# omuses/hqp

Hardware: AMD Instinct MI355X
Metric: KKT factor+solve/sec (fp64) (higher is better)
Workload: dtype f64; 1 GPU; C4 = BASELINE configs[3], the metric's 10^6-variable DOCP: multistage LQ optimal control QP, K=200 stages, nx=5000 states, nu=50 controls -> n=1015000 me=1005000 m=20000, dense fx/fu handed over as blocks, x_0 fixed, box bounds on u; plugin LQDOCP (STAGED engine), one system per GPU; stages=200, nx=5000, nu=50, n=1015000, me=1005000, m=20000, plugin=LQDOCP, kkt_dim_full=2040000

## Files before the change

### hqp_amd/_lib.py

```python
from __future__ import annotations

import ctypes as C
import os

import numpy as np

_HERE = os.path.dirname(os.path.abspath(__file__))
LIB_PATH = os.environ.get("HQPKKT_LIB") or os.path.join(_HERE, "libhqpkkt.so")

OK, E_SIZES, E_MEM, E_SING, E_FORMAT, E_NULL, E_RANGE, E_INTERN, E_DEVICE = 0, 1, 3, 4, 6, 8, 10, 17, 100
MODE_FULL, MODE_REDUCED, MODE_STAGED = 0, 1, 2
LOC_HOST, LOC_DEVICE = 0, 1
DYN_DENSE, DYN_SPARSE, DYN_PROFILE = 0, 1, 3
HESS_CSR, HESS_DENSE = 0, 1
HQPKKT_HESS_UPDATE_RANK = 4
HQPKKT_BFGS_REPORT = 8
HQPKKT_EIG_MAX_STEPS = 128
HQPKKT_EIG_REPORT = 10
HQPKKT_EIG_END_REL = 2.0 ** -40

SYMBOLS = [
    "hqpkkt_default_opts", "hqpkkt_create", "hqpkkt_destroy", "hqpkkt_analyze",
    "hqpkkt_set_values", "hqpkkt_factor", "hqpkkt_step", "hqpkkt_residual", "hqpkkt_solve",
    "hqpkkt_get_sbw", "hqpkkt_get_perm", "hqpkkt_set_tol", "hqpkkt_set_eps",
# ... 4 lines not shown
    "hqpkkt_set_stages", "hqpkkt_debug_stage_ranks", "hqpkkt_debug_stage_block", "hqpkkt_debug_dgemm", "hqpkkt_debug_dgemm2", "hqpkkt_debug_dgemm_full", "hqpkkt_debug_sk_table", "hqpkkt_debug_gemm_form",
    "hqpkkt_analyze_staged", "hqpkkt_set_values_staged", "hqpkkt_set_shard_stream",
    "hqpkkt_values_staging", "hqpkkt_detect_stages", "hqpkkt_stage_staging", "hqpkkt_set_stage_block",
    "hqpkkt_debug_factor_block", "hqpkkt_debug_solve_top_stamps", "hqpkkt_set_dynamics_form", "hqpkkt_set_dense_columns",
    "hqpkkt_debug_sk_profile", "hqpkkt_debug_gemv_profile",
    "hqpkkt_set_packed_panels", "hqpkkt_debug_dgemm_packed", "hqpkkt_debug_gemv_packed", "hqpkkt_debug_carried_packed",
    "hqpkkt_set_dense_rows", "hqpkkt_debug_dgemm_ctrl_rows", "hqpkkt_debug_sk_ctrl_rows",
    "hqpkkt_set_hessian_form", "hqpkkt_set_stage_hessian", "hqpkkt_debug_stage_hessian", "hqpkkt_debug_hess_symv",
    "hqpkkt_set_packed_hessians", "hqpkkt_debug_hess_symv_timed",
    "hqpkkt_update_stage_hessians", "hqpkkt_hessian_product",
    "hqpkkt_bfgs_update_stage_hessians", "hqpkkt_bfgs_report",
    "hqpkkt_hessian_row_stats", "hqpkkt_restart_stage_hessians", "hqpkkt_gerschgorin_stage_hessians",
    "hqpkkt_eigen_control_stage_hessians", "hqpkkt_eigen_report",
    "hqpkkt_debug_gemm_schedule",
    "hqpkkt_debug_gemv_dense", "hqpkkt_debug_symv", "hqpkkt_debug_symv_batch", "hqpkkt_debug_symv_map",
    "hqpkkt_debug_rows_gemv",
]
RCCL_LIB_PATH = os.path.join(_HERE, "libhqpkkt_rccl.so")
RCCL_SYMBOLS = ["hqpkkt_rccl_unique_id", "hqpkkt_rccl_create", "hqpkkt_rccl_create_from_env",
                "hqpkkt_rccl_comm_info", "hqpkkt_rccl_exchange", "hqpkkt_rccl_destroy", "hqpkkt_rccl_origin"]

XCHG_ALLGATHER, XCHG_ALLREDUCE_SUM, XCHG_BCAST_BASE = 0, 1, 16
EXCHANGE_FN = C.CFUNCTYPE(C.c_int, C.c_void_p, C.c_int, C.c_void_p, C.c_longlong, C.c_int)


class Opts(C.Structure):
    _fields_ = [("mode", C.c_int), ("device", C.c_int), ("loc", C.c_int), ("tol", C.c_double),
                ("eps", C.c_double), ("pivot_eps", C.c_double), ("leaf_size", C.c_int),
                ("max_pivots", C.c_int), ("zd_policy", C.c_int), ("slack_policy", C.c_int),
                ("no_small_fronts", C.c_int), ("upd_pingpong_mb", C.c_int), ("amalgamation", C.c_int),
                ("ordering", C.c_int)]
# ... 169 lines not shown
    L.hqpkkt_debug_stage_block.argtypes = [vp, C.c_int, vp, C.c_longlong, C.POINTER(C.c_longlong)]
    L.hqpkkt_debug_dgemm2.argtypes = [C.c_int] * 8 + [C.POINTER(C.c_double)] * 2 + [C.POINTER(C.c_longlong)]
    L.hqpkkt_debug_dgemm_full.argtypes = [C.c_int, C.POINTER(DgemmCase)]
    L.hqpkkt_debug_sk_table.argtypes = [C.c_longlong, C.c_int, C.c_int, C.c_int, C.POINTER(C.c_int), C.c_longlong, C.POINTER(C.c_longlong),
                                        C.POINTER(C.c_int), C.POINTER(C.c_int)]
    L.hqpkkt_debug_dgemm_ctrl_rows.argtypes = [C.c_int, C.POINTER(CtrlRowsCase)]
    L.hqpkkt_debug_sk_ctrl_rows.argtypes = [C.c_int] * 5 + [C.POINTER(C.c_int), C.c_longlong, C.POINTER(C.c_int), C.POINTER(C.c_longlong)]
    L.hqpkkt_debug_sk_profile.argtypes = [C.POINTER(C.c_int), C.c_longlong, C.c_int, C.POINTER(C.c_int), C.c_longlong, C.POINTER(C.c_longlong)]
    L.hqpkkt_debug_gemv_profile.argtypes = [C.c_int] * 4 + [vp, C.c_longlong, C.c_longlong, vp, vp, vp, C.c_double, vp]
    L.hqpkkt_debug_dgemm_packed.argtypes = [C.c_int, C.POINTER(DgemmCase), vp, C.c_longlong, vp]
    L.hqpkkt_debug_gemv_packed.argtypes = [C.c_int] * 4 + [vp, C.c_longlong, vp, vp, vp, vp, C.c_double, vp]
    L.hqpkkt_debug_carried_packed.argtypes = [C.c_int] * 4 + [vp, C.c_longlong, C.c_longlong, vp, C.c_longlong, vp, vp, vp] + [C.c_longlong] * 4
    L.hqpkkt_debug_gemm_form.argtypes = [C.c_int] * 7 + [C.c_longlong] * 3 + [C.c_int, C.POINTER(C.c_longlong)] + [C.POINTER(C.c_int)] * 3
    L.hqpkkt_debug_gemm_schedule.argtypes = [C.POINTER(GemmCaps), C.POINTER(GemmLaunch), C.POINTER(GemmLaunch), C.POINTER(GemmScheduleOut),
                                             C.POINTER(C.c_int), C.c_longlong, C.POINTER(C.c_int), C.c_longlong]
    L.hqpkkt_debug_gemv_dense.argtypes = [C.c_int, C.c_int, C.POINTER(GemvCase)]
    L.hqpkkt_debug_rows_gemv.argtypes = [C.c_int, C.c_int, C.POINTER(RowsCase)]
    L.hqpkkt_debug_symv.argtypes = [C.c_int, C.POINTER(GemvCase)]
    L.hqpkkt_debug_symv_batch.argtypes = [C.c_int, C.c_int, C.POINTER(GemvCase), vp, C.c_longlong, vp, C.c_longlong, C.c_int, C.c_int]
    L.hqpkkt_debug_symv_map.restype = C.c_longlong
    L.hqpkkt_debug_symv_map.argtypes = [C.c_int, C.POINTER(C.c_int), C.c_longlong]
    L.hqpkkt_debug_solve_top_stamps.argtypes = [vp, vp, C.c_int]
    L.hqpkkt_debug_factor_block.argtypes = [C.c_int, C.c_int, vp, C.c_double, C.c_double, C.c_int, C.c_int] + [vp] * 7
    _lib = L
    return L


_rccl = None


# ... 18 lines not shown
```

### hqp_amd/csrc/gemm_form.hpp

```cpp
#pragma once
#include <algorithm>

namespace stg {

static const int GEMM_BK = 16;

static inline long long gemm_tiles(int M, int N, int b, int lower) {
  const long long tm = (M + b - 1) / b, tn = (N + b - 1) / b;
  return lower ? tn * (tn + 1) / 2 + (tm > tn ? (tm - tn) * tn : 0) : tm * tn;
}
static inline long long gemm_slabs(int K) { return (K + GEMM_BK - 1) / GEMM_BK; }

static inline bool gemm_big_tiles(int M, int N, int lower, int K = 0) {
  const long long t = gemm_tiles(M, N, 128, lower);
  return t >= 384 || (!lower && t >= 160 && t <= 256 && K >= 256 * GEMM_BK);
}

static inline bool gemm_use_split_tiles(long long tiles, long long nslab, int grid) {
  if (grid <= 0 || nslab < 32) return false;
  return !(tiles % grid == 0 || tiles >= 16LL * grid);
}
static inline bool gemm_use_split(int M, int N, int K, int lower, int grid) {
  if ((long long)M * N < 256LL * 256) return false;
  const long long tiles = gemm_tiles(M, N, 128, lower);
  if (!gemm_use_split_tiles(tiles, gemm_slabs(K), grid)) return false;
  return tiles > grid * 5 / 8;
// ... 66 lines not shown
```

### hqp_amd/csrc/staged_gemm.hip.h

```cpp
#pragma once
#include <hip/hip_runtime.h>

#include <algorithm>
#include <vector>

#include "gemm_schedule.hpp"

namespace stg {

using kktdev::double4_t;
using kktdev::mfma_f64;

typedef double double2_t __attribute__((ext_vector_type(2)));

struct StripTab {
  int nranks;
  int cut[17];
  int ld[17];
  long long off[17];
};
struct RectTab {
  int nranks;
  int cut[17];
  struct Block {
// ... 52 lines not shown

__device__ __forceinline__ int xcd_swizzle(int bid, int nwg) {
  const int q = nwg >> 3, r = nwg & 7, x = bid & 7;
  return x * q + (x < r ? x : r) + (bid >> 3);
}

template <int BM, int BN, int WGM = 2, int WGN = 2>
struct GemmTile {
  static constexpr int BK = GEMM_BK;
  static constexpr int NW = WGM * WGN, NT = 64 * NW;
  static constexpr int LDA = BM + 16, LDB = BN + 16;
  static constexpr int WM = BM / WGM, WN = BN / WGN, TM = WM / 16, TN = WN / 16;
  static constexpr int LA = BK * BM / 2 / 256, LB = BK * BN / 2 / 256;
  static constexpr int RA = 256 / (BM / 2), RB = 256 / (BN / 2);

  static __device__ __forceinline__ void tile_of(const GemmArgs &g, int t, int &tm, int &tn) {
    if (g.tile_map && BM == 128) {
      const int e = g.tile_map[t];
      tm = e >> 16, tn = e & 0xffff;
    } else if (g.lower) {
      const int tcols = (g.N + BN - 1) / BN, tri = tcols * (tcols + 1) / 2;
      if (t < tri) {
        tm = (int)((sqrtf(8.0f * (float)t + 1.0f) - 1.0f) * 0.5f);
        while ((tm + 1) * (tm + 2) / 2 <= t) tm++;
        while (tm * (tm + 1) / 2 > t) tm--;
        tn = t - tm * (tm + 1) / 2;
      } else {
        tm = tcols + (t - tri) / tcols;
        tn = (t - tri) % tcols;
      }
// ... 106 lines not shown
      }
    }
  }

  static __device__ __forceinline__ void glds16(const double *src, double *lds_row) {
    __builtin_amdgcn_global_load_lds((const __attribute__((address_space(1))) void *)src,
                                     (__attribute__((address_space(3))) void *)lds_row, 16, 0, 0);
  }
  struct Rows {
    int K, k0, k1;
    long long ld, o2, ld2;
  };
  static __device__ __forceinline__ const double *row_of(const Rows &r, const double *p, const double *zr, int k) {
    return k < r.K ? p + (long long)k * r.ld : (k >= r.k0 && k < r.k1) ? p + (r.o2 + (long long)k * r.ld2) : zr;
  }
  template <bool MASKED>
  static __device__ __forceinline__ void slabs_dma(const Rows &ra, const Rows &rb, const double *pa, const double *pb, const double *zr, int wave,
                                                   int wm, int wn, int lr, int lk, int s0, int s1, unsigned mask,
                                                   double4_t (&acc)[TM][TN], double *As, double *Bs) {
    constexpr int RPW = BK / NW;
    auto dma = [&](int buf, int k0, int p) {
      const int r = wave + NW * (p % RPW), k = k0 + r;
      if (p < RPW)
        glds16(row_of(ra, pa, zr, k), As + (buf * BK + r) * LDA);
      else
        glds16(row_of(rb, pb, zr, k), Bs + (buf * BK + r) * LDB);
    };
    if (s1 > s0) {
#pragma unroll
      for (int p = 0; p < 2 * RPW; p++) dma(0, s0 * BK, p);
    }
    __syncthreads();
    constexpr int GAP = TM * TN / (2 * RPW);
    for (int s = s0; s < s1; s++) {
      const int buf = (s - s0) & 1;
      const int knext = s + 1 < s1 ? (s + 1) * BK : ra.k1;
      const double *Ab = As + buf * BK * LDA + wm * WM + lr;
      const double *Bb = Bs + buf * BK * LDB + wn * WN + lr;
#pragma unroll
      for (int ks = 0; ks < BK / 4; ks++) {
        double af[TM], bf[TN];
#pragma unroll
        for (int x = 0; x < TM; x++) af[x] = Ab[(ks * 4 + lk) * LDA + 16 * x];
#pragma unroll
        for (int y = 0; y < TN; y++) bf[y] = Bb[(ks * 4 + lk) * LDB + 16 * y];
#pragma unroll
        for (int x = 0; x < TM; x++)
#pragma unroll
          for (int y = 0; y < TN; y++) {
            if (!MASKED || ((mask >> (x * TN + y)) & 1u)) acc[x][y] = mfma_f64(af[x], bf[y], acc[x][y]);
            if (ks == 0 && (x * TN + y) % GAP == GAP - 1) dma(buf ^ 1, knext, (x * TN + y) / GAP);
          }
      }
      __syncthreads();
    }
  }
  template <bool MASKED>
  static __device__ __forceinline__ void slabs_dma3(const Rows &ra, const Rows &rb, const double *pa, const double *pb, const double *zr, int wave,
                                                    int wm, int wn, int lr, int lk, int s0, int s1, unsigned mask,
                                                    double4_t (&acc)[TM][TN], double *As, double *Bs) {
    constexpr int RPW = BK / NW;
    static_assert(2 * RPW == 4 || 2 * RPW == 8, "the counted waits below are written for 4 or 8 pieces per wave and slab");
    auto dma = [&](int buf, int k0, int p) {
      const int r = wave + NW * (p % RPW), k = k0 + r;
      if (p < RPW)
        glds16(row_of(ra, pa, zr, k), As + (buf * BK + r) * LDA);
      else
        glds16(row_of(rb, pb, zr, k), Bs + (buf * BK + r) * LDB);
    };
    auto wait_all_but_newest_slab = [&]() {
      if constexpr (2 * RPW == 4)
        asm volatile("s_waitcnt vmcnt(4) lgkmcnt(0)\n\ts_barrier" ::: "memory");
      else
        asm volatile("s_waitcnt vmcnt(8) lgkmcnt(0)\n\ts_barrier" ::: "memory");
    };
#pragma unroll
    for (int p = 0; p < 2 * RPW; p++) dma(0, s1 > s0 ? s0 * BK : ra.k1, p);
#pragma unroll
    for (int p = 0; p < 2 * RPW; p++) dma(1, s0 + 1 < s1 ? (s0 + 1) * BK : ra.k1, p);
    wait_all_but_newest_slab();
    constexpr int GAP = TM * TN / (2 * RPW);
    int buf = 0;
    for (int s = s0; s < s1; s++) {
      const int bnext = buf >= 1 ? buf - 1 : 2;
      const int knext = s + 2 < s1 ? (s + 2) * BK : ra.k1;
      const double *Ab = As + buf * BK * LDA + wm * WM + lr;
      const double *Bb = Bs + buf * BK * LDB + wn * WN + lr;
#pragma unroll
      for (int ks = 0; ks < BK / 4; ks++) {
        double af[TM], bf[TN];
#pragma unroll
        for (int x = 0; x < TM; x++) af[x] = Ab[(ks * 4 + lk) * LDA + 16 * x];
#pragma unroll
        for (int y = 0; y < TN; y++) bf[y] = Bb[(ks * 4 + lk) * LDB + 16 * y];
#pragma unroll
        for (int x = 0; x < TM; x++)
#pragma unroll
          for (int y = 0; y < TN; y++) {
            if (!MASKED || ((mask >> (x * TN + y)) & 1u)) acc[x][y] = mfma_f64(af[x], bf[y], acc[x][y]);
            if (ks == 0 && (x * TN + y) % GAP == GAP - 1) dma(bnext, knext, (x * TN + y) / GAP);
          }
      }
      wait_all_but_newest_slab();
      buf = buf == 2 ? 0 : buf + 1;
    }
    asm volatile("s_waitcnt vmcnt(0)" ::: "memory");
    __syncthreads();
  }
  template <bool PACKED = false>
  static __device__ __forceinline__ void accumulate_dma(const GemmArgs &g, int i0, int j0, int s0, int s1,
                                                        double4_t (&acc)[TM][TN], double *As, double *Bs, bool skip_upper = false, int nbuf = 2) {
    static_assert(BM == 128 && BN == 128, "one k-row of a panel must be one 1-KiB wave-instruction");
    static_assert((BK / NW) * NW == BK && TM * TN >= 2 * (BK / NW) && TM * TN <= 32,
                  "pieces are issued behind the multiplications of the first k-step");
    const int tid = threadIdx.x, lane = tid & 63, wave = __builtin_amdgcn_readfirstlane(tid >> 6);
    const int wm = wave / WGN, wn = wave % WGN;
    const int lr = lane & 15, lk = lane >> 4;
    unsigned mask = 0;
#pragma unroll
    for (int x = 0; x < TM; x++)
#pragma unroll
      for (int y = 0; y < TN; y++) {
        const int rb = wm * TM + x, cb = wn * TN + y;
        const bool want = i0 + 16 * rb < g.M && j0 + 16 * cb < g.N && !(skip_upper && cb > rb);
        mask |= (want ? 1u : 0u) << (x * TN + y);
      }
    mask = __builtin_amdgcn_readfirstlane(mask);
    const bool all = mask == (TM * TN == 32 ? 0xffffffffu : (1u << (TM * TN)) - 1u);
    const double *B = g.B;
    long long ldb = g.ldb;
    int jb = j0;
    if (g.bstrips) {
      const int q = strip_of(g.bstrips->cut, g.bstrips->nranks, j0);
      B = g.B + g.bstrips->off[q], ldb = g.bstrips->ld[q], jb = j0 - g.bstrips->cut[q];
    }
    const double *A = g.A;
    long long lda = g.lda;
    int ia = i0;
    if constexpr (PACKED) {
      if (g.apack) A = g.A + g.apack[i0 / BM].off, lda = g.apack[i0 / BM].ld, ia = 0;
      if (g.bpack) B = g.B + g.bpack[j0 / BN].off, ldb = g.bpack[j0 / BN].ld, jb = 0;
    }
    const double *pa = A + ((ia + 2 * lane < lda) ? ia + 2 * lane : 0);
    const double *pb = B + ((jb + 2 * lane < ldb) ? jb + 2 * lane : 0);
    const double *zr = g.zeros + 2 * lane;
    const int k0 = (g.K + BK - 1) / BK * BK, k1 = k0 + (g.K2 > 0 ? g.K2 : 0);
    Rows ra{g.K, k0, k1, lda, 0, 0}, rb{g.K, k0, k1, ldb, 0, 0};
    if (g.K2 > 0) {
      ra.ld2 = g.lda2, ra.o2 = (g.A2 - g.A) - (long long)k0 * g.lda2;
      rb.ld2 = g.ldb2, rb.o2 = (g.B2 - g.B) - (long long)k0 * g.ldb2;
    }
    if (nbuf == 3) {
      if (all)
        slabs_dma3<false>(ra, rb, pa, pb, zr, wave, wm, wn, lr, lk, s0, s1, mask, acc, As, Bs);
      else
        slabs_dma3<true>(ra, rb, pa, pb, zr, wave, wm, wn, lr, lk, s0, s1, mask, acc, As, Bs);
    } else if (all)
      slabs_dma<false>(ra, rb, pa, pb, zr, wave, wm, wn, lr, lk, s0, s1, mask, acc, As, Bs);
    else
      slabs_dma<true>(ra, rb, pa, pb, zr, wave, wm, wn, lr, lk, s0, s1, mask, acc, As, Bs);
  }

  static __device__ __forceinline__ void accumulate_dma_aug(const GemmArgs &g, int i0, int j0, int s0, int s1, bool ready,
                                                            double4_t (&acc)[TM][TN], double *As, double *Bs, int nbuf) {
    static_assert(BM == 128 && BN == 128, "one k-row of a panel must be one 1-KiB wave-instruction");
    const int tid = threadIdx.x, lane = tid & 63, wave = __builtin_amdgcn_readfirstlane(tid >> 6);
    const int wm = wave / WGN, wn = wave % WGN;
    const int lr = lane & 15, lk = lane >> 4;
    const int r = g.M - i0, rows = ready ? r + g.mu : r;
    unsigned mask = 0;
#pragma unroll
    for (int x = 0; x < TM; x++)
#pragma unroll
      for (int y = 0; y < TN; y++) {
        const int rb = wm * TM + x, cb = wn * TN + y;
        mask |= ((16 * rb < rows && j0 + 16 * cb < g.N) ? 1u : 0u) << (x * TN + y);
      }
    mask = __builtin_amdgcn_readfirstlane(mask);
    const double *zr = g.zeros + 2 * lane;
    const int c = 2 * lane;
    const bool mine = c < r, theirs = !mine && c < rows;
    const double *pa = mine ? g.A + ((i0 + c < g.lda) ? i0 + c : 0) : theirs ? g.Au + (c - r) : zr;
    const double *pb = g.B + ((j0 + c < g.ldb) ? j0 + c : 0);
    const int k0 = (g.K + BK - 1) / BK * BK;
    const Rows ra{g.K, k0, k0, mine ? g.lda : theirs ? g.ldau : 0, 0, 0}, rb{g.K, k0, k0, g.ldb, 0, 0};
    if (nbuf == 3)
      slabs_dma3<true>(ra, rb, pa, pb, zr, wave, wm, wn, lr, lk, s0, s1, mask, acc, As, Bs);
    else
      slabs_dma<true>(ra, rb, pa, pb, zr, wave, wm, wn, lr, lk, s0, s1, mask, acc, As, Bs);
  }
  static __device__ __forceinline__ void epilogue_aug(const GemmArgs &g, int tm, int tn, const double4_t (&acc)[TM][TN], bool plain, bool ctrl) {
    const int tid = threadIdx.x, lane = tid & 63, wave = tid >> 6;
    const int wm = wave / WGN, wn = wave % WGN;
    const int lr = lane & 15, lk = lane >> 4;
    const int i0 = tm * BM, j0 = tn * BN, r = g.M - i0;
#pragma unroll
    for (int x = 0; x < TM; x++)
#pragma unroll
      for (int y = 0; y < TN; y++)
#pragma unroll
        for (int rg = 0; rg < 4; rg++) {
          const int ii = wm * WM + 16 * x + lk + 4 * rg, j = j0 + wn * WN + 16 * y + lr;
          if (j >= g.N) continue;
          const double v = g.alpha * acc[x][y][rg];
          if (ii < r) {
            if (plain) g.C[(long long)(i0 + ii) * g.ldc + j] = v;
          } else if (ii < r + g.mu && ctrl)
            g.Cu[(long long)(ii - r) * g.ldcu + j] = v;
        }
  }

  static __device__ __forceinline__ void epilogue(const GemmArgs &g, int tm, int tn, const double4_t (&acc)[TM][TN], double *lds) {
    const int tid = threadIdx.x, lane = tid & 63, wave = tid >> 6;
    const int wm = wave / WGN, wn = wave % WGN;
    const int lr = lane & 15, lk = lane >> 4;
    const int i0 = tm * BM, j0 = tn * BN;
    const bool diag = g.lower && tm == tn;
    const double *cin = g.Cin;
    long long ldcin = g.ldcin;
    if (g.rects && g.beta != 0.0) {
      const RectTab &R = *g.rects;
      const int a = strip_of(R.cut, R.nranks, i0), b = strip_of(R.cut, R.nranks, j0);
      const RectTab::Block &blk = R.blk[a * 16 + b];
      const int t = i0 >= blk.rsplit ? 1 : 0, r0 = t ? blk.rsplit : R.cut[a], c0 = R.cut[b];
      ldcin = R.cut[b + 1] - c0;
      cin = g.Cin + blk.off[t] - ((long long)r0 * ldcin + c0);
    }
    constexpr int HC = BN < 64 ? BN : 64, LDT = BM + 2;
    const bool via_lds = g.mirror && !diag && lds != nullptr;
    double4_t val[TM][TN];
#pragma unroll
    for (int x = 0; x < TM; x++)
#pragma unroll
      for (int y = 0; y < TN; y++)
#pragma unroll
        for (int rg = 0; rg < 4; rg++) {
          const int i = i0 + wm * WM + 16 * x + lk + 4 * rg, j = j0 + wn * WN + 16 * y + lr;
          double v = 0.0;
          if (i < g.M && j < g.N && !(diag && i < j)) {
            v = g.alpha * acc[x][y][rg];
            if (g.beta != 0.0) v += g.beta * cin[(long long)i * ldcin + j];
            g.C[(long long)i * g.ldc + j] = v;
            if (g.mirror && i != j && !via_lds) g.C[(long long)j * g.ldc + i] = v;
          }
          val[x][y][rg] = v;
        }
    if (via_lds) {
#pragma unroll
      for (int h = 0; h < BN / HC; h++) {
        if ((wn * WN) / HC == h) {
#pragma unroll
          for (int x = 0; x < TM; x++)
#pragma unroll
            for (int y = 0; y < TN; y++)
#pragma unroll
              for (int rg = 0; rg < 4; rg++)
                lds[(wn * WN - h * HC + 16 * y + lr) * LDT + wm * WM + 16 * x + lk + 4 * rg] = val[x][y][rg];
        }
        __syncthreads();
        for (int jj = wave; jj < HC; jj += NW) {
          const int j = j0 + h * HC + jj;
          if (j >= g.N) break;
          for (int ii = 2 * lane; ii < BM; ii += 128) {
            const int i = i0 + ii;
            double *dst = g.C + (long long)j * g.ldc + i;
            if (i + 1 < g.M && (((size_t)dst) & 15) == 0)
              *(double2_t *)dst = *(const double2_t *)(lds + jj * LDT + ii);
            else {
              if (i < g.M) dst[0] = lds[jj * LDT + ii];
              if (i + 1 < g.M) dst[1] = lds[jj * LDT + ii + 1];
            }
          }
// ... 354 lines not shown
```

### hqp_amd/csrc/staged_hooks.hip.h

```cpp
#pragma once

extern "C" {

namespace {
__global__ void k_fill_rand(double *p, long long n, unsigned long long seed) {
  long long i = (long long)blockIdx.x * blockDim.x + threadIdx.x;
  if (i >= n) return;
  unsigned long long x = (unsigned long long)i * 0x9E3779B97F4A7C15ULL + seed;
  x ^= x >> 30, x *= 0xBF58476D1CE4E5B9ULL, x ^= x >> 27, x *= 0x94D049BB133111EBULL, x ^= x >> 31;
  p[i] = (double)(x >> 11) * (1.0 / 9007199254740992.0) - 0.5;
}
__global__ void k_gemm_check(stg::GemmArgs g, int nsample, double *err) {
  const int sidx = blockIdx.x * blockDim.x + threadIdx.x;
  if (sidx >= nsample) return;
  unsigned long long x = (unsigned long long)sidx * 0x9E3779B97F4A7C15ULL + 12345;
  x ^= x >> 29, x *= 0xBF58476D1CE4E5B9ULL, x ^= x >> 32;
  int i = (int)(x % (unsigned long long)g.M), j = (int)((x >> 20) % (unsigned long long)g.N);
  int ci = i, cj = j;
  if (g.lower && i < j) {
    const int t = i;
    i = j, j = t;
    if (!g.mirror) ci = i, cj = j;
  }
  double s = 0.0, sa = 0.0;
// ... 7 lines not shown
  }
  const double e = fabs(g.C[(long long)ci * g.ldc + cj] - g.alpha * s) / (sa + 1e-300);
  atomic_max_pos((unsigned long long *)err, e);
}
__global__ void k_negate_into(long long n, const double *__restrict__ x, double *__restrict__ y) {
  const long long i = (long long)blockIdx.x * blockDim.x + threadIdx.x;
  if (i < n) y[i] = -x[i];
}
__global__ void k_gemm_count_asym(stg::GemmArgs g, unsigned long long *count) {
  const long long e = (long long)blockIdx.x * blockDim.x + threadIdx.x;
  if (e >= (long long)g.M * g.N) return;
  const int i = (int)(e / g.N), j = (int)(e % g.N);
  if (i <= j || i >= g.N) return;
  if (__double_as_longlong(g.C[(long long)i * g.ldc + j]) != __double_as_longlong(g.C[(long long)j * g.ldc + i])) atomicAdd(count, 1ULL);
}
static void dgemm_stamps_split(const stg::GemmArgs &g, const stg::GemmForm &f, int variant, int skg, int list, const stg::SplitTable &sk_tab, const stg::SkUnit *tab_dev) {
  DBuf<unsigned long long> st;
  DBuf<double> ws2;
  DBuf<unsigned> cnt2;
  if (st.alloc(32 * (size_t)skg) || ws2.alloc((size_t)std::max<long long>(sk_tab.pieces, 1) * 128 * 128) || cnt2.alloc(f.tiles + 4)) return;
  (void)hipMemset(st.p, 0, sizeof(unsigned long long) * 32 * skg);
  (void)hipMemset(cnt2.p, 0, sizeof(unsigned) * (f.tiles + 4));
  stg::GemmArgs gs = g;
  gs.stamps = st.p;
  stg::gemm_launch_split(variant, skg, 0, gs, stg::SplitPlan{ws2.p, cnt2.p, tab_dev, sk_tab.stride});
  std::vector<unsigned long long> hs(32 * (size_t)skg);
  if (hipMemcpy(hs.data(), st.p, sizeof(unsigned long long) * 32 * skg, hipMemcpyDeviceToHost) != hipSuccess) return;
  unsigned long long tmin = ~0ULL;
  for (int w = 0; w < skg; w++) tmin = std::min(tmin, hs[32 * (size_t)w]);
  fprintf(stderr, "%s shares: %lld parked pieces", list == stg::SK_LIST_UNEQUAL ? "unequal" : "equal", sk_tab.pieces);
  if (list == stg::SK_LIST_UNEQUAL) fprintf(stderr, ", %d / %d whole tiles per first / second workgroup of a CU", sk_tab.nA, sk_tab.nB);
// ... 10 lines not shown
    }
    fprintf(stderr, "\n");
  }
  for (int c = 0; c < 2; c++) {
    double lo = 1e30, hi = 0.0, sum = 0.0;
    int n = 0;
    for (int w = c * skg / 2; w < (c + 1) * skg / 2; w++) {
      unsigned long long last = 0;
      for (int r = 0; r < 10; r++) last = std::max(last, hs[32 * (size_t)w + 3 * r + 3]);
      if (!last) continue;
      const double e = (last - tmin) * 0.01;
      lo = std::min(lo, e), hi = std::max(hi, e), sum += e, n++;
    }
    if (n) fprintf(stderr, "  class %c (blockIdx %s grid / 2): last epilogue ends at %.1f ... %.1f us, mean %.1f\n", c ? 'B' : 'A', c ? ">=" : "<", lo, hi, sum / n);
  }
}
static void dgemm_stamps_plain(const stg::GemmArgs &g, long long tiles, int variant) {
  DBuf<unsigned long long> st;
  if (st.alloc(4 * (size_t)tiles)) return;
  stg::GemmArgs gs = g;
  gs.stamps = st.p;
  stg::gemm_launch_plain(variant, (unsigned)tiles, 0, gs);
  std::vector<unsigned long long> hs(4 * tiles);
  if (hipMemcpy(hs.data(), st.p, sizeof(unsigned long long) * 4 * tiles, hipMemcpyDeviceToHost) != hipSuccess) return;
  unsigned long long tmin = ~0ULL;
  for (long long t = 0; t < tiles; t++) tmin = std::min(tmin, hs[4 * t]);
  std::vector<long long> ord(tiles);
  for (long long t = 0; t < tiles; t++) ord[t] = t;
  std::sort(ord.begin(), ord.end(), [&](long long a, long long b) { return hs[4 * a] < hs[4 * b]; });
  fprintf(stderr, "stamps (us after the first start; %lld workgroups, every %lldth in start order): start, k loop end, epilogue end, xcc, blockIdx\n", tiles,
// ... 104 lines not shown
  (void)hipEventCreate(&e0.h), (void)hipEventCreate(&e1.h);
  for (int r = -1; r < reps; r++) {
    if (r == 0) (void)hipEventRecord(e0, 0);
    run.launch(g);
  }
  (void)hipEventRecord(e1, 0);
  hipError_t se = hipDeviceSynchronize();
  if (mu > 0 && run.ctl.p) fprintf(stderr, "control-row segment: %d of %d launches fell back\n", run.fallbacks(), reps + 1);
  run.ws.release(), run.cnt.release();
  float t = 0.f;
  (void)hipEventElapsedTime(&t, e0, e1);
  if (se != hipSuccess) return HQPKKT_E_DEVICE;
  if (getenv("HQPKKT_DGEMM_STAMPS")) {
    const stg::GemmSchedule &sc = run.e->s;
    const stg::GemmArgs gc = stg::gemm_complete(sc, stg::GemmBufs{nullptr, run.e->order.p, nullptr, nullptr, nullptr, run.zr.p}, g);
    if (sc.f.kind == stg::GEMM_FORM_CUT) dgemm_stamps_split(gc, sc.f, sc.variant, run.caps.grid, sc.list, sc.tab, run.e->units.p);
    if (sc.f.kind == stg::GEMM_FORM_PLAIN) dgemm_stamps_plain(gc, sc.f.tiles, sc.variant);
  }
  k_gemm_check<<<16, 256>>>(g, 4096, err.p);
  double he = 0.0;
  if (hipMemcpy(&he, err.p, 8, hipMemcpyDeviceToHost) != hipSuccess) return HQPKKT_E_DEVICE;
  if (asym) {
    unsigned long long na = 0;
    if (nasym.alloc(1)) return HQPKKT_E_MEM;
    (void)hipMemset(nasym.p, 0, 8);
    if (lower && mirror) k_gemm_count_asym<<<nblk((long long)M * N), 256>>>(g, nasym.p);
    if (hipMemcpy(&na, nasym.p, 8, hipMemcpyDeviceToHost) != hipSuccess) return HQPKKT_E_DEVICE;
    *asym = (long long)na;
  }
  if (ms) *ms = t / reps;
  if (max_err) *max_err = he;
// ... 168 lines not shown
    if (status == stg::GEMM_SCHED_OK && order) std::copy(s.order.begin(), s.order.end(), order);
    return status;
  });
}

int hqpkkt_debug_sk_table(long long tiles, int nslab, int grid, int kind, int *units, long long cap_ints, long long *pieces, int *whole_a, int *whole_b) {
  stg::SplitTable t;
  if (!stg::gemm_list_table(kind, tiles, nslab, grid, t)) return 0;
  if (pieces) *pieces = t.pieces;
  if (whole_a) *whole_a = t.nA;
  if (whole_b) *whole_b = t.nB;
  if (!units_out(t, units, cap_ints)) return 0;
  return t.stride;
}

int hqpkkt_debug_sk_profile(const int *ranges, long long tiles, int grid, int *units, long long cap_ints, long long *pieces) {
  stg::SplitTable t;
  if (!stg::gemm_profile_table(ranges, tiles, grid, t)) return 0;
  if (pieces) *pieces = t.pieces;
  if (!units_out(t, units, cap_ints)) return 0;
  return t.stride;
}

static int debug_gemv_profile(int device, int rows_form, int K, int N, const double *A, long long a_rows, long long ld, const int *ranges,
                              const double *x, const double *add, double alpha, double *y, const long long *panel = nullptr) {
  if (!A || !ranges || !x || !y) return HQPKKT_E_NULL;
  if (K <= 0 || N <= 0 || (!panel && (a_rows < K || ld < N || (ld & 7)))) return HQPKKT_E_RANGE;
  std::vector<stg::PackPanel> ptab;
  if (panel && (a_rows < 1 || ld < 1 || debug_pack_table(K, N, panel, ranges, a_rows * ld, ptab))) return HQPKKT_E_RANGE;
  const int np = (N + 127) / 128, nx = rows_form ? N : K, ny = rows_form ? K : N;
// ... 374 lines not shown
```

### include/hqpkkt.h

```cpp
#ifndef HQPKKT_H
#define HQPKKT_H

#ifdef __cplusplus
extern "C" {
#endif

#define HQPKKT_VERSION 1

#define HQPKKT_OK 0
#define HQPKKT_E_SIZES 1
#define HQPKKT_E_MEM 3
#define HQPKKT_E_SING 4
#define HQPKKT_E_FORMAT 6
#define HQPKKT_E_NULL 8
#define HQPKKT_E_RANGE 10
#define HQPKKT_E_INTERN 17
#define HQPKKT_E_DEVICE 100

#define HQPKKT_MODE_FULL 0
#define HQPKKT_MODE_REDUCED 1
#define HQPKKT_MODE_STAGED 2

#define HQPKKT_LOC_HOST 0
#define HQPKKT_LOC_DEVICE 1
// ... 178 lines not shown
  int M, N, mu, grid;
  hqpkkt_dgemm_operand A, B;
  double *C;
  long long c_rows, ldc;
  double *Cu;
  long long cu_rows, ldcu;
  int taken, fallbacks, form;
  long long tiles;
} hqpkkt_ctrl_rows_case;
int hqpkkt_debug_dgemm_ctrl_rows(int device, hqpkkt_ctrl_rows_case *c);

int hqpkkt_debug_sk_ctrl_rows(int tiles_m, int tiles_n, int nslab, int grid, int kind, int *units, long long cap_ints, int *tile_map, long long *pieces);

int hqpkkt_debug_sk_table(long long tiles, int nslab, int grid, int kind, int *units, long long cap_ints, long long *pieces, int *whole_a, int *whole_b);

int hqpkkt_debug_sk_profile(const int *ranges, long long tiles, int grid, int *units, long long cap_ints, long long *pieces);

int hqpkkt_debug_gemv_profile(int device, int rows_form, int K, int N, const double *A, long long a_rows, long long ld, const int *ranges,
                              const double *x, const double *add, double alpha, double *y);

int hqpkkt_debug_dgemm_packed(int device, hqpkkt_dgemm_case *c, const double *packed, long long packed_elems, const long long *panel);
int hqpkkt_debug_gemv_packed(int device, int rows_form, int K, int N, const double *packed, long long packed_elems, const long long *panel,
                             const int *ranges, const double *x, const double *add, double alpha, double *y);
int hqpkkt_debug_carried_packed(int device, int K, int N, int R, const double *BT, long long bt_rows, long long ldb, const double *packed,
                                long long packed_elems, const long long *panel, const int *ranges, double *C, long long c_rows, long long ldc,
                                long long c_row0, long long c_col0);

typedef struct hqpkkt_gemv_case {
  int M, N;
  hqpkkt_dgemm_operand A, A2;
// ... 101 lines not shown
```

Before: 0.8483 KKT factor+solve/s.

## Remap wave column blocks on diagonal and edge tiles, specialize masked MFMA paths

On diagonal tiles of lower-triangular GEMMs and on last-column partial tiles, each wave's two 16-column blocks are remapped (wn and 7-wn) so that the useful MFMA work is spread evenly across waves instead of piling onto a few. Common mask patterns are also dispatched to compile-time-specialized slab loops, so the per-MFMA mask test is resolved statically. The epilogue and LDS mirror write are updated to follow the remapped columns, and a debug entry point plus per-tile-kind timing stats are added. The cost is more template instantiations, which grows code size and may raise register pressure.

New measurement: 0.8485 KKT factor+solve/s, median of 2. Within noise of the previous version (+0.0%).

```diff
diff --git a/hqp_amd/_lib.py b/hqp_amd/_lib.py
--- a/hqp_amd/_lib.py
+++ b/hqp_amd/_lib.py
@@ -42,7 +42,7 @@
     "hqpkkt_eigen_control_stage_hessians", "hqpkkt_eigen_report",
     "hqpkkt_debug_gemm_schedule",
     "hqpkkt_debug_gemv_dense", "hqpkkt_debug_symv", "hqpkkt_debug_symv_batch", "hqpkkt_debug_symv_map",
-    "hqpkkt_debug_rows_gemv",
+    "hqpkkt_debug_rows_gemv", "hqpkkt_debug_gemm_col_block",
 ]
 RCCL_LIB_PATH = os.path.join(_HERE, "libhqpkkt_rccl.so")
 RCCL_SYMBOLS = ["hqpkkt_rccl_unique_id", "hqpkkt_rccl_create", "hqpkkt_rccl_create_from_env",
@@ -242,6 +242,7 @@
     L.hqpkkt_debug_gemm_form.argtypes = [C.c_int] * 7 + [C.c_longlong] * 3 + [C.c_int, C.POINTER(C.c_longlong)] + [C.POINTER(C.c_int)] * 3
     L.hqpkkt_debug_gemm_schedule.argtypes = [C.POINTER(GemmCaps), C.POINTER(GemmLaunch), C.POINTER(GemmLaunch), C.POINTER(GemmScheduleOut),
                                              C.POINTER(C.c_int), C.c_longlong, C.POINTER(C.c_int), C.c_longlong]
+    L.hqpkkt_debug_gemm_col_block.argtypes = [C.c_int] * 6 + [C.POINTER(C.c_int)]
     L.hqpkkt_debug_gemv_dense.argtypes = [C.c_int, C.c_int, C.POINTER(GemvCase)]
     L.hqpkkt_debug_rows_gemv.argtypes = [C.c_int, C.c_int, C.POINTER(RowsCase)]
     L.hqpkkt_debug_symv.argtypes = [C.c_int, C.POINTER(GemvCase)]
diff --git a/hqp_amd/csrc/gemm_form.hpp b/hqp_amd/csrc/gemm_form.hpp
--- a/hqp_amd/csrc/gemm_form.hpp
+++ b/hqp_amd/csrc/gemm_form.hpp
@@ -10,6 +10,9 @@
   return lower ? tn * (tn + 1) / 2 + (tm > tn ? (tm - tn) * tn : 0) : tm * tn;
 }
 static inline long long gemm_slabs(int K) { return (K + GEMM_BK - 1) / GEMM_BK; }
+
+constexpr bool gemm_tile_remapped(int N, int lower, int tm, int tn) { return (lower && tm == tn) || tn * 128 + 112 >= N; }
+constexpr int gemm_col_block(bool remapped, int wgn, int tn, int wn, int y) { return remapped ? (y == 0 ? wn : wgn * tn - 1 - wn) : wn * tn + y; }
 
 static inline bool gemm_big_tiles(int M, int N, int lower, int K = 0) {
   const long long t = gemm_tiles(M, N, 128, lower);
diff --git a/hqp_amd/csrc/staged_gemm.hip.h b/hqp_amd/csrc/staged_gemm.hip.h
--- a/hqp_amd/csrc/staged_gemm.hip.h
+++ b/hqp_amd/csrc/staged_gemm.hip.h
@@ -90,6 +90,12 @@
   static constexpr int LA = BK * BM / 2 / 256, LB = BK * BN / 2 / 256;
   static constexpr int RA = 256 / (BM / 2), RB = 256 / (BN / 2);
 
+  static constexpr bool REMAP = BM == 128 && BN == 128 && WGN == 4 && TN == 2;
+  static __device__ __forceinline__ bool remapped(const GemmArgs &g, int i0, int j0) {
+    return REMAP && gemm_tile_remapped(g.N, g.lower, i0 / BM, j0 / BN);
+  }
+  static __device__ __forceinline__ int col_block(bool remap, int wn, int y) { return gemm_col_block(REMAP && remap, WGN, TN, wn, y); }
+
   static __device__ __forceinline__ void tile_of(const GemmArgs &g, int t, int &tm, int &tn) {
     if (g.tile_map && BM == 128) {
       const int e = g.tile_map[t];
@@ -226,10 +232,11 @@
   static __device__ __forceinline__ const double *row_of(const Rows &r, const double *p, const double *zr, int k) {
     return k < r.K ? p + (long long)k * r.ld : (k >= r.k0 && k < r.k1) ? p + (r.o2 + (long long)k * r.ld2) : zr;
   }
-  template <bool MASKED>
+  static constexpr unsigned NO_CM = ~0u;
+  template <bool MASKED, unsigned CM = NO_CM>
   static __device__ __forceinline__ void slabs_dma(const Rows &ra, const Rows &rb, const double *pa, const double *pb, const double *zr, int wave,
                                                    int wm, int wn, int lr, int lk, int s0, int s1, unsigned mask,
-                                                   double4_t (&acc)[TM][TN], double *As, double *Bs) {
+                                                   int b0, int bstep, double4_t (&acc)[TM][TN], double *As, double *Bs) {
     constexpr int RPW = BK / NW;
     auto dma = [&](int buf, int k0, int p) {
       const int r = wave + NW * (p % RPW), k = k0 + r;
@@ -248,29 +255,29 @@
       const int buf = (s - s0) & 1;
       const int knext = s + 1 < s1 ? (s + 1) * BK : ra.k1;
       const double *Ab = As + buf * BK * LDA + wm * WM + lr;
-      const double *Bb = Bs + buf * BK * LDB + wn * WN + lr;
+      const double *Bb = Bs + buf * BK * LDB + (MASKED ? b0 : wn * WN) + lr;
 #pragma unroll
       for (int ks = 0; ks < BK / 4; ks++) {
         double af[TM], bf[TN];
 #pragma unroll
         for (int x = 0; x < TM; x++) af[x] = Ab[(ks * 4 + lk) * LDA + 16 * x];
 #pragma unroll
-        for (int y = 0; y < TN; y++) bf[y] = Bb[(ks * 4 + lk) * LDB + 16 * y];
+        for (int y = 0; y < TN; y++) bf[y] = Bb[(ks * 4 + lk) * LDB + (MASKED ? bstep : 16) * y];
 #pragma unroll
         for (int x = 0; x < TM; x++)
 #pragma unroll
           for (int y = 0; y < TN; y++) {
-            if (!MASKED || ((mask >> (x * TN + y)) & 1u)) acc[x][y] = mfma_f64(af[x], bf[y], acc[x][y]);
+            if (!MASKED || (((CM != NO_CM ? CM : mask) >> (x * TN + y)) & 1u)) acc[x][y] = mfma_f64(af[x], bf[y], acc[x][y]);
             if (ks == 0 && (x * TN + y) % GAP == GAP - 1) dma(buf ^ 1, knext, (x * TN + y) / GAP);
           }
       }
       __syncthreads();
     }
   }
-  template <bool MASKED>
+  template <bool MASKED, unsigned CM = NO_CM>
   static __device__ __forceinline__ void slabs_dma3(const Rows &ra, const Rows &rb, const double *pa, const double *pb, const double *zr, int wave,
                                                     int wm, int wn, int lr, int lk, int s0, int s1, unsigned mask,
-                                                    double4_t (&acc)[TM][TN], double *As, double *Bs) {
+                                                    int b0, int bstep, double4_t (&acc)[TM][TN], double *As, double *Bs) {
     constexpr int RPW = BK / NW;
     static_assert(2 * RPW == 4 || 2 * RPW == 8, "the counted waits below are written for 4 or 8 pieces per wave and slab");
     auto dma = [&](int buf, int k0, int p) {
@@ -297,19 +304,19 @@
       const int bnext = buf >= 1 ? buf - 1 : 2;
       const int knext = s + 2 < s1 ? (s + 2) * BK : ra.k1;
       const double *Ab = As + buf * BK * LDA + wm * WM + lr;
-      const double *Bb = Bs + buf * BK * LDB + wn * WN + lr;
+      const double *Bb = Bs + buf * BK * LDB + (MASKED ? b0 : wn * WN) + lr;
 #pragma unroll
       for (int ks = 0; ks < BK / 4; ks++) {
         double af[TM], bf[TN];
 #pragma unroll
         for (int x = 0; x < TM; x++) af[x] = Ab[(ks * 4 + lk) * LDA + 16 * x];
 #pragma unroll
-        for (int y = 0; y < TN; y++) bf[y] = Bb[(ks * 4 + lk) * LDB + 16 * y];
+        for (int y = 0; y < TN; y++) bf[y] = Bb[(ks * 4 + lk) * LDB + (MASKED ? bstep : 16) * y];
 #pragma unroll
         for (int x = 0; x < TM; x++)
 #pragma unroll
           for (int y = 0; y < TN; y++) {
-            if (!MASKED || ((mask >> (x * TN + y)) & 1u)) acc[x][y] = mfma_f64(af[x], bf[y], acc[x][y]);
+            if (!MASKED || (((CM != NO_CM ? CM : mask) >> (x * TN + y)) & 1u)) acc[x][y] = mfma_f64(af[x], bf[y], acc[x][y]);
             if (ks == 0 && (x * TN + y) % GAP == GAP - 1) dma(bnext, knext, (x * TN + y) / GAP);
           }
       }
@@ -318,6 +325,39 @@
     }
     asm volatile("s_waitcnt vmcnt(0)" ::: "memory");
     __syncthreads();
+  }
+  template <unsigned CM>
+  static __device__ __forceinline__ void slabs_masked_as(int nbuf, const Rows &ra, const Rows &rb, const double *pa, const double *pb, const double *zr, int wave,
+                                                         int wm, int wn, int lr, int lk, int s0, int s1, unsigned mask, int b0, int bstep,
+                                                         double4_t (&acc)[TM][TN], double *As, double *Bs) {
+    if (nbuf == 3)
+      slabs_dma3<true, CM>(ra, rb, pa, pb, zr, wave, wm, wn, lr, lk, s0, s1, mask, b0, bstep, acc, As, Bs);
+    else
+      slabs_dma<true, CM>(ra, rb, pa, pb, zr, wave, wm, wn, lr, lk, s0, s1, mask, b0, bstep, acc, As, Bs);
+  }
+  static __device__ __forceinline__ void slabs_masked(int nbuf, const Rows &ra, const Rows &rb, const double *pa, const double *pb, const double *zr, int wave,
+                                                      int wm, int wn, int lr, int lk, int s0, int s1, unsigned mask, int b0, int bstep,
+                                                      double4_t (&acc)[TM][TN], double *As, double *Bs) {
+#define HQPKKT_MASK_CASE(CM) \
+  case CM: return slabs_masked_as<CM>(nbuf, ra, rb, pa, pb, zr, wave, wm, wn, lr, lk, s0, s1, mask, b0, bstep, acc, As, Bs)
+    if constexpr (TM == 4 && TN == 2) {
+      switch (mask) {
+        HQPKKT_MASK_CASE(0x00u);
+        HQPKKT_MASK_CASE(0x01u);
+        HQPKKT_MASK_CASE(0x03u);
+        HQPKKT_MASK_CASE(0x55u);
+        HQPKKT_MASK_CASE(0x54u);
+        HQPKKT_MASK_CASE(0x50u);
+        HQPKKT_MASK_CASE(0x40u);
+        HQPKKT_MASK_CASE(0xd5u);
+        HQPKKT_MASK_CASE(0xf5u);
+        HQPKKT_MASK_CASE(0xfdu);
+        HQPKKT_MASK_CASE(0xffu);
+        default: break;
+      }
+    }
+#undef HQPKKT_MASK_CASE
+    slabs_masked_as<NO_CM>(nbuf, ra, rb, pa, pb, zr, wave, wm, wn, lr, lk, s0, s1, mask, b0, bstep, acc, As, Bs);
   }
   template <bool PACKED = false>
   static __device__ __forceinline__ void accumulate_dma(const GemmArgs &g, int i0, int j0, int s0, int s1,
@@ -328,17 +368,19 @@
     const int tid = threadIdx.x, lane = tid & 63, wave = __builtin_amdgcn_readfirstlane(tid >> 6);
     const int wm = wave / WGN, wn = wave % WGN;
     const int lr = lane & 15, lk = lane >> 4;
+    const bool remap = remapped(g, i0, j0);
     unsigned mask = 0;
 #pragma unroll
     for (int x = 0; x < TM; x++)
 #pragma unroll
       for (int y = 0; y < TN; y++) {
-        const int rb = wm * TM + x, cb = wn * TN + y;
+        const int rb = wm * TM + x, cb = col_block(remap, wn, y);
         const bool want = i0 + 16 * rb < g.M && j0 + 16 * cb < g.N && !(skip_upper && cb > rb);
         mask |= (want ? 1u : 0u) << (x * TN + y);
       }
     mask = __builtin_amdgcn_readfirstlane(mask);
-    const bool all = mask == (TM * TN == 32 ? 0xffffffffu : (1u << (TM * TN)) - 1u);
+    const bool all = !remap && mask == (TM * TN == 32 ? 0xffffffffu : (1u << (TM * TN)) - 1u);
+    const int b0 = 16 * col_block(remap, wn, 0), bstep = TN > 1 ? 16 * (col_block(remap, wn, 1) - col_block(remap, wn, 0)) : 16;
     const double *B = g.B;
     long long ldb = g.ldb;
     int jb = j0;
@@ -362,15 +404,12 @@
       ra.ld2 = g.lda2, ra.o2 = (g.A2 - g.A) - (long long)k0 * g.lda2;
       rb.ld2 = g.ldb2, rb.o2 = (g.B2 - g.B) - (long long)k0 * g.ldb2;
     }
-    if (nbuf == 3) {
-      if (all)
-        slabs_dma3<false>(ra, rb, pa, pb, zr, wave, wm, wn, lr, lk, s0, s1, mask, acc, As, Bs);
-      else
-        slabs_dma3<true>(ra, rb, pa, pb, zr, wave, wm, wn, lr, lk, s0, s1, mask, acc, As, Bs);
-    } else if (all)
-      slabs_dma<false>(ra, rb, pa, pb, zr, wave, wm, wn, lr, lk, s0, s1, mask, acc, As, Bs);
+    if (!all)
+      slabs_masked(nbuf, ra, rb, pa, pb, zr, wave, wm, wn, lr, lk, s0, s1, mask, b0, bstep, acc, As, Bs);
+    else if (nbuf == 3)
+      slabs_dma3<false>(ra, rb, pa, pb, zr, wave, wm, wn, lr, lk, s0, s1, mask, b0, bstep, acc, As, Bs);
     else
-      slabs_dma<true>(ra, rb, pa, pb, zr, wave, wm, wn, lr, lk, s0, s1, mask, acc, As, Bs);
+      slabs_dma<false>(ra, rb, pa, pb, zr, wave, wm, wn, lr, lk, s0, s1, mask, b0, bstep, acc, As, Bs);
   }
 
   static __device__ __forceinline__ void accumulate_dma_aug(const GemmArgs &g, int i0, int j0, int s0, int s1, bool ready,
@@ -380,15 +419,17 @@
     const int wm = wave / WGN, wn = wave % WGN;
     const int lr = lane & 15, lk = lane >> 4;
     const int r = g.M - i0, rows = ready ? r + g.mu : r;
+    const bool remap = remapped(g, i0, j0);
     unsigned mask = 0;
 #pragma unroll
     for (int x = 0; x < TM; x++)
 #pragma unroll
       for (int y = 0; y < TN; y++) {
-        const int rb = wm * TM + x, cb = wn * TN + y;
+        const int rb = wm * TM + x, cb = col_block(remap, wn, y);
         mask |= ((16 * rb < rows && j0 + 16 * cb < g.N) ? 1u : 0u) << (x * TN + y);
       }
     mask = __builtin_amdgcn_readfirstlane(mask);
+    const int b0 = 16 * col_block(remap, wn, 0), bstep = TN > 1 ? 16 * (col_block(remap, wn, 1) - col_block(remap, wn, 0)) : 16;
     const double *zr = g.zeros + 2 * lane;
     const int c = 2 * lane;
     const bool mine = c < r, theirs = !mine && c < rows;
@@ -396,23 +437,21 @@
     const double *pb = g.B + ((j0 + c < g.ldb) ? j0 + c : 0);
     const int k0 = (g.K + BK - 1) / BK * BK;
     const Rows ra{g.K, k0, k0, mine ? g.lda : theirs ? g.ldau : 0, 0, 0}, rb{g.K, k0, k0, g.ldb, 0, 0};
-    if (nbuf == 3)
-      slabs_dma3<true>(ra, rb, pa, pb, zr, wave, wm, wn, lr, lk, s0, s1, mask, acc, As, Bs);
-    else
-      slabs_dma<true>(ra, rb, pa, pb, zr, wave, wm, wn, lr, lk, s0, s1, mask, acc, As, Bs);
+    slabs_masked(nbuf, ra, rb, pa, pb, zr, wave, wm, wn, lr, lk, s0, s1, mask, b0, bstep, acc, As, Bs);
   }
   static __device__ __forceinline__ void epilogue_aug(const GemmArgs &g, int tm, int tn, const double4_t (&acc)[TM][TN], bool plain, bool ctrl) {
     const int tid = threadIdx.x, lane = tid & 63, wave = tid >> 6;
     const int wm = wave / WGN, wn = wave % WGN;
     const int lr = lane & 15, lk = lane >> 4;
     const int i0 = tm * BM, j0 = tn * BN, r = g.M - i0;
+    const bool remap = remapped(g, i0, j0);
 #pragma unroll
     for (int x = 0; x < TM; x++)
 #pragma unroll
       for (int y = 0; y < TN; y++)
 #pragma unroll
         for (int rg = 0; rg < 4; rg++) {
-          const int ii = wm * WM + 16 * x + lk + 4 * rg, j = j0 + wn * WN + 16 * y + lr;
+          const int ii = wm * WM + 16 * x + lk + 4 * rg, j = j0 + 16 * col_block(remap, wn, y) + lr;
           if (j >= g.N) continue;
           const double v = g.alpha * acc[x][y][rg];
           if (ii < r) {
@@ -440,6 +479,7 @@
     }
     constexpr int HC = BN < 64 ? BN : 64, LDT = BM + 2;
     const bool via_lds = g.mirror && !diag && lds != nullptr;
+    const bool remap = remapped(g, i0, j0);
     double4_t val[TM][TN];
 #pragma unroll
     for (int x = 0; x < TM; x++)
@@ -447,7 +487,7 @@
       for (int y = 0; y < TN; y++)
 #pragma unroll
         for (int rg = 0; rg < 4; rg++) {
-          const int i = i0 + wm * WM + 16 * x + lk + 4 * rg, j = j0 + wn * WN + 16 * y + lr;
+          const int i = i0 + wm * WM + 16 * x + lk + 4 * rg, j = j0 + 16 * col_block(remap, wn, y) + lr;
           double v = 0.0;
           if (i < g.M && j < g.N && !(diag && i < j)) {
             v = g.alpha * acc[x][y][rg];
@@ -460,14 +500,15 @@
     if (via_lds) {
 #pragma unroll
       for (int h = 0; h < BN / HC; h++) {
-        if ((wn * WN) / HC == h) {
-#pragma unroll
-          for (int x = 0; x < TM; x++)
-#pragma unroll
-            for (int y = 0; y < TN; y++)
-#pragma unroll
-              for (int rg = 0; rg < 4; rg++)
-                lds[(wn * WN - h * HC + 16 * y + lr) * LDT + wm * WM + 16 * x + lk + 4 * rg] = val[x][y][rg];
+#pragma unroll
+        for (int y = 0; y < TN; y++) {
+          const int c0 = 16 * col_block(remap, wn, y);
+          if (c0 / HC == h) {
+#pragma unroll
+            for (int x = 0; x < TM; x++)
+#pragma unroll
+              for (int rg = 0; rg < 4; rg++) lds[(c0 - h * HC + lr) * LDT + wm * WM + 16 * x + lk + 4 * rg] = val[x][y][rg];
+          }
         }
         __syncthreads();
         for (int jj = wave; jj < HC; jj += NW) {
diff --git a/hqp_amd/csrc/staged_hooks.hip.h b/hqp_amd/csrc/staged_hooks.hip.h
--- a/hqp_amd/csrc/staged_hooks.hip.h
+++ b/hqp_amd/csrc/staged_hooks.hip.h
@@ -45,7 +45,8 @@
   if (i <= j || i >= g.N) return;
   if (__double_as_longlong(g.C[(long long)i * g.ldc + j]) != __double_as_longlong(g.C[(long long)j * g.ldc + i])) atomicAdd(count, 1ULL);
 }
-static void dgemm_stamps_split(const stg::GemmArgs &g, const stg::GemmForm &f, int variant, int skg, int list, const stg::SplitTable &sk_tab, const stg::SkUnit *tab_dev) {
+static void dgemm_stamps_split(const stg::GemmArgs &g, const stg::GemmForm &f, int variant, int skg, int list, const stg::SplitTable &sk_tab, const stg::SkUnit *tab_dev,
+                               const int *order) {
   DBuf<unsigned long long> st;
   DBuf<double> ws2;
   DBuf<unsigned> cnt2;
@@ -86,6 +87,49 @@
     }
     if (n) fprintf(stderr, "  class %c (blockIdx %s grid / 2): last epilogue ends at %.1f ... %.1f us, mean %.1f\n", c ? 'B' : 'A', c ? ">=" : "<", lo, hi, sum / n);
   }
+  static const char *const kinds[] = {"full", "diagonal", "last row", "last column", "corner", "last row + segment", "corner + segment"};
+  const int TM = (g.M + 127) / 128, TN = (g.N + 127) / 128, nslab = stg::gemm_slabs_of(g);
+  std::vector<double> whole[7][2], slab[2];
+  for (int w = 0; w < skg; w++)
+    for (int r = 0; r < nr; r++) {
+      const stg::SkUnit &u = sk_tab.units[(size_t)w * sk_tab.stride + r];
+      if (u.tile < 0) break;
+      const unsigned long long t0 = r ? hs[32 * (size_t)w + 3 * r] : hs[32 * (size_t)w], t1 = hs[32 * (size_t)w + 3 * r + 3];
+      if (!t1 || t1 < t0) continue;
+      const double us = (t1 - t0) * 0.01;
+      int tm, tn;
+      bool aug = false;
+      if (g.Au && order) {
+        const int e = order[u.tile];
+        aug = e < 0, tm = (e >> 16) & 0x7fff, tn = e & 0xffff;
+      } else
+        stg::gemm_tile_of_host(g.M, g.N, g.lower, order, u.tile, tm, tn);
+      const bool lrow = tm == TM - 1 && (g.M & 127), lcol = tn == TN - 1 && (g.N & 127), diag = g.lower && tm == tn;
+      const int kind = aug ? (lcol ? 6 : 5) : (lrow && (lcol || diag)) ? 4 : diag ? 1 : lrow ? 2 : lcol ? 3 : 0;
+      const int cls = w < skg / 2 ? 0 : 1;
+      if (u.pieces == 1 && u.s1 - u.s0 == nslab)
+        whole[kind][cls].push_back(us);
+      else if (kind == 0 && u.s1 > u.s0)
+        slab[cls].push_back(us / (u.s1 - u.s0) * nslab);
+    }
+  auto stat = [&](const char *name, int cls, std::vector<double> &v, double full) {
+    if (v.empty()) return;
+    std::sort(v.begin(), v.end());
+    const double med = v[v.size() / 2];
+    fprintf(stderr, "  %-20s class %c: n %4zu  min %7.1f  median %7.1f  max %7.1f us", name, cls ? 'B' : 'A', v.size(), v.front(), med, v.back());
+    if (full > 0.0) fprintf(stderr, "  = %.2f of a full tile", med / full);
+    fprintf(stderr, "\n");
+  };
+  fprintf(stderr, "  whole tiles of %d slabs by kind (a unit: end of the one before it -> end of its epilogue):\n", nslab);
+  double full[2] = {0.0, 0.0};
+  for (int c = 0; c < 2; c++)
+    if (!whole[0][c].empty()) {
+      std::sort(whole[0][c].begin(), whole[0][c].end());
+      full[c] = whole[0][c][whole[0][c].size() / 2];
+    }
+  for (int k = 0; k < 7; k++)
+    for (int c = 0; c < 2; c++) stat(kinds[k], c, whole[k][c], k ? full[c] : 0.0);
+  for (int c = 0; c < 2; c++) stat("pieces of full tiles (x slabs)", c, slab[c], full[c]);
 }
 static void dgemm_stamps_plain(const stg::GemmArgs &g, long long tiles, int variant) {
   DBuf<unsigned long long> st;
@@ -220,7 +264,7 @@
   if (getenv("HQPKKT_DGEMM_STAMPS")) {
     const stg::GemmSchedule &sc = run.e->s;
     const stg::GemmArgs gc = stg::gemm_complete(sc, stg::GemmBufs{nullptr, run.e->order.p, nullptr, nullptr, nullptr, run.zr.p}, g);
-    if (sc.f.kind == stg::GEMM_FORM_CUT) dgemm_stamps_split(gc, sc.f, sc.variant, run.caps.grid, sc.list, sc.tab, run.e->units.p);
+    if (sc.f.kind == stg::GEMM_FORM_CUT) dgemm_stamps_split(gc, sc.f, sc.variant, run.caps.grid, sc.list, sc.tab, run.e->units.p, sc.order.empty() ? nullptr : sc.order.data());
     if (sc.f.kind == stg::GEMM_FORM_PLAIN) dgemm_stamps_plain(gc, sc.f.tiles, sc.variant);
   }
   k_gemm_check<<<16, 256>>>(g, 4096, err.p);
@@ -419,6 +463,13 @@
   return t.stride;
 }
 
+int hqpkkt_debug_gemm_col_block(int N, int lower, int tm, int tn, int wn, int y, int *remapped) {
+  if (N <= 0 || tm < 0 || tn < 0 || wn < 0 || wn > 3 || y < 0 || y > 1) return -1;
+  const bool re = stg::gemm_tile_remapped(N, lower, tm, tn);
+  if (remapped) *remapped = re ? 1 : 0;
+  return stg::gemm_col_block(re, 4, 2, wn, y);
+}
+
 int hqpkkt_debug_sk_profile(const int *ranges, long long tiles, int grid, int *units, long long cap_ints, long long *pieces) {
   stg::SplitTable t;
   if (!stg::gemm_profile_table(ranges, tiles, grid, t)) return 0;
diff --git a/include/hqpkkt.h b/include/hqpkkt.h
--- a/include/hqpkkt.h
+++ b/include/hqpkkt.h
@@ -216,6 +216,8 @@
 
 int hqpkkt_debug_sk_table(long long tiles, int nslab, int grid, int kind, int *units, long long cap_ints, long long *pieces, int *whole_a, int *whole_b);
 
+int hqpkkt_debug_gemm_col_block(int N, int lower, int tm, int tn, int wn, int y, int *remapped);
+
 int hqpkkt_debug_sk_profile(const int *ranges, long long tiles, int grid, int *units, long long cap_ints, long long *pieces);
 
 int hqpkkt_debug_gemv_profile(int device, int rows_form, int K, int N, const double *A, long long a_rows, long long ld, const int *ranges,
```
